# OpenNLPLab/ACR_WSSS

Measured on AMD Instinct MI355X. Metric: img/s ACR-ViT-hybrid-base 448x448 train step, higher is better.
Workload: dtype f32_split; 1 GPU; BASELINE configs[1]: ViT-hybrid-base (DPT) 448x448, batch 16 per GPU, ACR train step (2 views, fwd+bwd+SGD); global_batch=16, classes=20, alpha=125, parallelism=dp1

## Files before the change

acr_wsss_amd/csrc/gemm_f32.hip:

```cpp
#include <math.h>

#include <mutex>
#include <type_traits>
#include <unordered_map>

#include "acr_common.h"

typedef __bf16 bf16_t;

#define F_BM 128
#define F_BN 128
#define F_BK 32
#define F_PKC 36
#define F_PKS 128
#define F_STAGE (F_BM * F_PKC)

struct GemmF32Args {
    const float* a; int64_t lda;
    const float* b; int64_t ldb;
    const float* bias;
    const float* aux; int64_t ldaux;
    float* c; int64_t ldc;
    float* c2;
    float* cs;
    int M, N, K;
    int tiles_m, tiles_n, nsplit, kps;
    int tile0, tiles_launch;
    int nkb_a, nkb_b;
    int img_nkb;
    const int* ea; const int* eb;
    int64_t a_zs, b_zs, c_zs, aux_zs;
    int k_zs, ksplit;
};

#define F_BAND 8
__device__ __forceinline__ void tile_coords(int tt, int tiles_m, int tiles_n, int& tm, int& tn) {
    const int per_band = F_BAND * tiles_n;
    const int band = tt / per_band, in_band = tt - band * per_band;
    const int first = band * F_BAND;
    const int rows = min(tiles_m - first, F_BAND);
    tn = in_band / rows;
    tm = first + (in_band - tn * rows);
}

template <bool KC>
__device__ __forceinline__ void load_chunk(f32x4 (&r)[4], const float* __restrict__ p, int64_t ld, int i0, int dim, int k0,
                                           int kend, int tid) {
#pragma unroll
    for (int ps = 0; ps < 4; ++ps) {
        const int f = tid + 256 * ps;
        if (KC) {
            const int i = min(i0 + (f >> 3), dim - 1), k = min(k0 + 4 * (f & 7), kend - 4);
            r[ps] = *reinterpret_cast<const f32x4*>(p + (int64_t)i * ld + k);
        } else {
            const int k = min(k0 + (f >> 5), kend - 1), i = min(i0 + 4 * (f & 31), dim - 4);
            r[ps] = *reinterpret_cast<const f32x4*>(p + (int64_t)k * ld + i);
        }
    }
}

template <bool KC>
__device__ __forceinline__ void store_chunk(float* __restrict__ s, f32x4 (&r)[4], int k0, int kend, int tid) {
    const f32x4 z = {0.f, 0.f, 0.f, 0.f};
#pragma unroll
    for (int ps = 0; ps < 4; ++ps) {
        const int f = tid + 256 * ps;
        if (KC) {
            if (k0 + 4 * (f & 7) >= kend) r[ps] = z;
            *reinterpret_cast<f32x4*>(s + (f >> 3) * F_PKC + 4 * (f & 7)) = r[ps];
        } else {
            if (k0 + (f >> 5) >= kend) r[ps] = z;
            *reinterpret_cast<f32x4*>(s + (f >> 5) * F_PKS + 4 * (f & 31)) = r[ps];
        }
    }
}

template <bool KC>
__device__ __forceinline__ f32x4 read_frag(const float* __restrict__ s, int base, int q, int r, int h) {
    if (KC) return *reinterpret_cast<const f32x4*>(s + (base + r) * F_PKC + 8 * q + 4 * h);
    const float* p = s + (8 * q + 4 * h) * F_PKS + base + r;
    f32x4 v = {p[0], p[F_PKS], p[2 * F_PKS], p[3 * F_PKS]};
    return v;
}

template <int ACT, bool EDGE>
__device__ __forceinline__ void epilogue_f32(const GemmF32Args& g, f32x16 (&acc)[2][2], int mb, int nb, int r, int h) {
#pragma unroll
    for (int j = 0; j < 2; ++j) {
        const int col = nb + j * 32 + r;
        const bool cok = !EDGE || col < g.N;
        const float bj = (ACT != 2 && g.bias && cok) ? g.bias[col] : 0.f;
#pragma unroll
        for (int i = 0; i < 2; ++i) {
            float x[16];
            if (ACT == 2 || (ACT == 0 && g.aux)) {
#pragma unroll
                for (int e = 0; e < 16; ++e) {
                    const int row = mb + i * 32 + acr_krow(e, h);
                    x[e] = (!EDGE || (row < g.M && cok)) ? g.aux[(int64_t)row * g.ldaux + col] : 0.f;
                }
            }
#pragma unroll
            for (int e = 0; e < 16; ++e) {
                const int row = mb + i * 32 + acr_krow(e, h);
                if (EDGE && !(row < g.M && cok)) continue;
                float v = acc[i][j][e] + bj;
                float* cp = g.c + (int64_t)row * g.ldc + col;
                if (ACT == 0) {
                    *cp = g.aux ? v + x[e] : v;
                } else if (ACT == 1) {
                    const float er = erff(v * 0.70710678118654752440f);
                    g.c2[(int64_t)row * g.ldc + col] = v * 0.5f * (1.0f + er);
                    *cp = 0.5f * (1.0f + er) + v * (expf(-0.5f * v * v) * 0.39894228040143267794f);
                } else {
                    *cp = v * x[e];
                }
            }
        }
    }
}

template <bool A_KC, bool B_KC, int ACT>
__global__ __launch_bounds__(256, 2) void gemm_f32_kernel(const GemmF32Args g) {
    __shared__ __attribute__((aligned(16))) float smem[4 * F_STAGE];
    const int tid = threadIdx.x, lane = tid & 63, wave = tid >> 6;
    const int r = lane & 31, h = lane >> 5, wm = wave >> 1, wn = wave & 1;
    const int ntile = g.tiles_launch;
    const int t = acr_xcd_remap(blockIdx.x, ntile * g.nsplit);
    const int split = t / ntile, tt = g.tile0 + (t - split * ntile);
    int tm, tn;
    if (ACT == 3) { tm = tt / g.tiles_n; tn = tt - tm * g.tiles_n; }
    else tile_coords(tt, g.tiles_m, g.tiles_n, tm, tn);
    const int m0 = tm * F_BM, n0 = tn * F_BN;
    const int zs = split / g.ksplit;
    const int kbeg = (split - zs * g.ksplit) * g.k_zs, kend = min(g.K, kbeg + g.kps);
    const float* __restrict__ pa = g.a + (int64_t)zs * g.a_zs;
    const float* __restrict__ pb = g.b + (int64_t)zs * g.b_zs;

    f32x16 acc[2][2];
#pragma unroll
    for (int i = 0; i < 2; ++i)
#pragma unroll
        for (int j = 0; j < 2; ++j)
#pragma unroll
            for (int e = 0; e < 16; ++e) acc[i][j][e] = 0.f;

    f32x4 ra0[4], rb0[4], ra1[4], rb1[4];
    float csum[4] = {0.f, 0.f, 0.f, 0.f};
    const bool want_cs = ACT == 3 && !A_KC && g.cs && tn == 0;
    auto add_cs = [&](f32x4 (&x)[4]) {
#pragma unroll
        for (int ps = 0; ps < 4; ++ps)
#pragma unroll
            for (int e = 0; e < 4; ++e) csum[e] += x[ps][e];
    };
    auto compute = [&](int buf) {
        const float* sa = smem + buf * 2 * F_STAGE;
        const float* sb = sa + F_STAGE;
#pragma unroll
        for (int q = 0; q < 4; ++q) {
            f32x4 av[2], bv[2];
#pragma unroll
            for (int i = 0; i < 2; ++i) av[i] = read_frag<A_KC>(sa, wm * 64 + i * 32, q, r, h);
#pragma unroll
            for (int j = 0; j < 2; ++j) bv[j] = read_frag<B_KC>(sb, wn * 64 + j * 32, q, r, h);
#pragma unroll
            for (int s = 0; s < 4; ++s)
#pragma unroll
                for (int i = 0; i < 2; ++i)
#pragma unroll
                    for (int j = 0; j < 2; ++j)
                        acc[i][j] = __builtin_amdgcn_mfma_f32_32x32x2f32(av[i][s], bv[j][s], acc[i][j], 0, 0, 0);
        }
    };
    auto step = [&](f32x4 (&la)[4], f32x4 (&lb)[4], f32x4 (&sa_)[4], f32x4 (&sb_)[4], int k0, int buf) {
        if (k0 + 2 * F_BK < kend) {
            load_chunk<A_KC>(la, pa, g.lda, m0, g.M, k0 + 2 * F_BK, kend, tid);
            load_chunk<B_KC>(lb, pb, g.ldb, n0, g.N, k0 + 2 * F_BK, kend, tid);
        }
        compute(buf);
        if (k0 + F_BK < kend) {
            float* d = smem + (buf ^ 1) * 2 * F_STAGE;
            store_chunk<A_KC>(d, sa_, k0 + F_BK, kend, tid);
            store_chunk<B_KC>(d + F_STAGE, sb_, k0 + F_BK, kend, tid);
            if (want_cs) add_cs(sa_);
        }
        __syncthreads();
    };
    load_chunk<A_KC>(ra0, pa, g.lda, m0, g.M, kbeg, kend, tid);
    load_chunk<B_KC>(rb0, pb, g.ldb, n0, g.N, kbeg, kend, tid);
    if (kbeg + F_BK < kend) {
        load_chunk<A_KC>(ra1, pa, g.lda, m0, g.M, kbeg + F_BK, kend, tid);
        load_chunk<B_KC>(rb1, pb, g.ldb, n0, g.N, kbeg + F_BK, kend, tid);
    }
    store_chunk<A_KC>(smem, ra0, kbeg, kend, tid);
    store_chunk<B_KC>(smem + F_STAGE, rb0, kbeg, kend, tid);
    if (want_cs) add_cs(ra0);
    __syncthreads();
    for (int k0 = kbeg; k0 < kend; k0 += 2 * F_BK) {
        step(ra0, rb0, ra1, rb1, k0, 0);
        if (k0 + F_BK < kend) step(ra1, rb1, ra0, rb0, k0 + F_BK, 1);
    }

    if (ACT == 3) {
        float* slab = g.c + (int64_t)split * g.M * g.ldc;
#pragma unroll
        for (int i = 0; i < 2; ++i)
#pragma unroll
            for (int j = 0; j < 2; ++j) {
                const int col = n0 + wn * 64 + j * 32 + r;
#pragma unroll
                for (int e = 0; e < 16; ++e) {
                    const int row = m0 + wm * 64 + i * 32 + acr_krow(e, h);
                    if (row < g.M && col < g.N) slab[(int64_t)row * g.ldc + col] = acc[i][j][e];
                }
            }
        if (!A_KC && g.cs && tn == 0) {
            float* red = smem;
            *reinterpret_cast<f32x4*>(red + (tid >> 5) * 128 + 4 * (tid & 31)) = *reinterpret_cast<f32x4*>(csum);
            __syncthreads();
            if (tid < 128) {
                float s = 0.f;
#pragma unroll
                for (int kr = 0; kr < 8; ++kr) s += red[kr * 128 + tid];
                if (m0 + tid < g.M) g.cs[(int64_t)split * g.M + m0 + tid] = s;
            }
        }
        return;
    }
    GemmF32Args gz = g;
    gz.c += (int64_t)zs * g.c_zs;
    if (gz.aux) gz.aux += (int64_t)zs * g.aux_zs;
    if (m0 + F_BM <= g.M && n0 + F_BN <= g.N)
        epilogue_f32<ACT, false>(gz, acc, m0 + wm * 64, n0 + wn * 64, r, h);
    else
        epilogue_f32<ACT, true>(gz, acc, m0 + wm * 64, n0 + wn * 64, r, h);
}


#define F_DTILE (F_BM * F_BK)

template <bool KC>
__device__ __forceinline__ void dma_offsets(int (&off)[4], int64_t ld, int i0, int dim, int wave, int lane) {
#pragma unroll
    for (int i = 0; i < 4; ++i) {
        const int piece = wave * 4 + i;
        if (KC) {
            const int row = piece * 8 + (lane >> 3);
            const int lc = (lane & 7) ^ ((row >> 1) & 7);
            off[i] = min(i0 + row, dim - 1) * (int)ld + lc * 4;
        } else {
            const int kr = piece * 2 + (lane >> 5);
            off[i] = kr * (int)ld + min(i0 + 4 * (lane & 31), dim - 4);
        }
    }
}
__device__ __forceinline__ void dma_chunk(float* s, const float* __restrict__ ub, const int (&off)[4], int wave) {
    typedef __attribute__((address_space(3))) void* lds_vp;
    typedef const __attribute__((address_space(1))) void* glb_vp;
#pragma unroll
    for (int i = 0; i < 4; ++i)
        __builtin_amdgcn_global_load_lds((glb_vp)(ub + off[i]), (lds_vp)(s + (wave * 4 + i) * 256), 16, 0, 0);
}

template <bool KC>
__device__ __forceinline__ f32x4 dma_frag(const float* __restrict__ s, int base, int q, int r, int h) {
    if (KC) {
        const int row = base + r;
        return *reinterpret_cast<const f32x4*>(s + row * F_BK + (((2 * q + h) ^ ((row >> 1) & 7)) << 2));
    }
    const float* p = s + (8 * q + 4 * h) * F_BM + base + r;
    f32x4 v = {p[0], p[F_BM], p[2 * F_BM], p[3 * F_BM]};
    return v;
}


template <bool A_KC, int ACT>
__device__ __forceinline__ void gemm_f32_finish(const GemmF32Args& g, f32x16 (&acc)[2][2], float* smem, int split, int tt, int tn, int m0,
                                                int n0, int zs, int wm, int wn, int r, int h, int tid, float csum, bool want_cs) {
    if (ACT == 4) {
        float* slab = g.c + ((int64_t)split * g.tiles_launch + (tt - g.tile0)) * (F_BM * F_BN);
#pragma unroll
        for (int i = 0; i < 2; ++i)
#pragma unroll
            for (int j = 0; j < 2; ++j) {
                const int col = wn * 64 + j * 32 + r;
#pragma unroll
                for (int e = 0; e < 16; ++e) slab[(wm * 64 + i * 32 + acr_krow(e, h)) * F_BN + col] = acc[i][j][e];
            }
        return;
    }
    if (ACT == 3) {
        float* slab = g.c + (int64_t)split * g.M * g.ldc;
#pragma unroll
        for (int i = 0; i < 2; ++i)
#pragma unroll
            for (int j = 0; j < 2; ++j) {
                const int col = n0 + wn * 64 + j * 32 + r;
#pragma unroll
                for (int e = 0; e < 16; ++e) {
                    const int row = m0 + wm * 64 + i * 32 + acr_krow(e, h);
                    if (row < g.M && col < g.N) slab[(int64_t)row * g.ldc + col] = acc[i][j][e];
                }
            }
        if (want_cs) {
            float* red = smem;
            red[tid] = csum;
            __syncthreads();
            if (tid < 128 && m0 + tid < g.M) g.cs[(int64_t)split * g.M + m0 + tid] = red[tid] + red[tid + 128];
        }
        return;
    }
    GemmF32Args gz = g;
    gz.c += (int64_t)zs * g.c_zs;
    if (gz.aux) gz.aux += (int64_t)zs * g.aux_zs;
    if (m0 + F_BM <= g.M && n0 + F_BN <= g.N)
        epilogue_f32<ACT, false>(gz, acc, m0 + wm * 64, n0 + wn * 64, r, h);
    else
        epilogue_f32<ACT, true>(gz, acc, m0 + wm * 64, n0 + wn * 64, r, h);
}

template <bool A_KC, bool B_KC, int ACT>
__global__ __launch_bounds__(256, 2) void gemm_f32_dma_kernel(const GemmF32Args g) {
    __shared__ __attribute__((aligned(1024))) float smem[4 * F_DTILE];
    const int tid = threadIdx.x, lane = tid & 63;
    const int wave = __builtin_amdgcn_readfirstlane(tid >> 6);
    const int r = lane & 31, h = lane >> 5, wm = wave >> 1, wn = wave & 1;
    const int ntile = g.tiles_launch;
    const int t = acr_xcd_remap(blockIdx.x, ntile * g.nsplit);
    const int split = t / ntile, tt = g.tile0 + (t - split * ntile);
    int tm, tn;
    if (ACT == 3) { tm = tt / g.tiles_n; tn = tt - tm * g.tiles_n; }
    else tile_coords(tt, g.tiles_m, g.tiles_n, tm, tn);
    const int m0 = tm * F_BM, n0 = tn * F_BN;
    const int zs = split / g.ksplit;
    const int kbeg = (split - zs * g.ksplit) * g.k_zs, kend = min(g.K, kbeg + g.kps);
    const float* __restrict__ pa = g.a + (int64_t)zs * g.a_zs;
    const float* __restrict__ pb = g.b + (int64_t)zs * g.b_zs;
    f32x16 acc[2][2];
#pragma unroll
    for (int i = 0; i < 2; ++i)
#pragma unroll
        for (int j = 0; j < 2; ++j)
#pragma unroll
            for (int e = 0; e < 16; ++e) acc[i][j][e] = 0.f;
    float csum = 0.f;
    const bool want_cs = ACT == 3 && !A_KC && g.cs && tn == 0;

    int offa[4], offb[4];
    dma_offsets<A_KC>(offa, g.lda, m0, g.M, wave, lane);
    dma_offsets<B_KC>(offb, g.ldb, n0, g.N, wave, lane);
    const int64_t ka = A_KC ? 1 : g.lda, kb = B_KC ? 1 : g.ldb;
    dma_chunk(smem, pa + kbeg * ka, offa, wave);
    dma_chunk(smem + F_DTILE, pb + kbeg * kb, offb, wave);
    acr_dma_barrier();
    int cur = 0;
    for (int k0 = kbeg; k0 < kend; k0 += F_BK, cur ^= 1) {
        if (k0 + F_BK < kend) {
            float* d = smem + (cur ^ 1) * 2 * F_DTILE;
            dma_chunk(d, pa + (k0 + F_BK) * ka, offa, wave);
            dma_chunk(d + F_DTILE, pb + (k0 + F_BK) * kb, offb, wave);
        }
// ... 517 lines not shown
    for (int i = 0; i < 2 * NP; ++i) {
        const int q = (wave & 1) * 2 * NP + i, pl = q >> 2, fs = min(f0 + 2 * (q & 3) + (lane >> 5), nkb - 1);
        offd[i] = (fs * NP + pl) * P_TILE_B + (lane & 31) * 16;
    }
    f32x16 acc[2][2];
#pragma unroll
    for (int i = 0; i < 2; ++i)
#pragma unroll
        for (int j = 0; j < 2; ++j)
#pragma unroll
            for (int e = 0; e < 16; ++e) acc[i][j][e] = 0.f;
    const int nst = (kend - kbeg) / P_BK;
    char* sm = reinterpret_cast<char*>(smem);
    auto dma1 = [&](int st, int slot, int i) {
        const int tk = kbeg + st * P_BK;
        const char* src = pw + ((int64_t)(tk >> 7) * nkb) * (NP * P_TILE_B) + (tk & 127) * 32;
        const int q = (wave & 1) * 2 * NP + i;
        __builtin_amdgcn_global_load_lds((glb_vp)(src + offd[i]), (lds_vp)(sm + slot * STAGE_B + (wave >> 1) * (NP * P_TILE_B) + (q >> 2) * P_TILE_B + (q & 3) * 1024),
                                         16, 0, 0);
    };
    const uint32_t lbase = (uint32_t)(uintptr_t)(const __attribute__((address_space(3))) char*)sm;
    const int i16 = lane & 15, g1 = (lane >> 4) & 1, qq = i16 >> 2, pp = i16 & 3;
    const uint32_t tlo = (4 * h + qq) * 32 + ((pp >> 1) << 4) + 8 * (pp & 1), thi = (8 + 4 * h + qq) * 32 + (((pp >> 1) ^ 1) << 4) + 8 * (pp & 1);
    const uint32_t fa_lo = lbase + (wm * 4 + g1) * 512 + tlo, fa_hi = lbase + (wm * 4 + g1) * 512 + thi;
    const uint32_t fb_lo = lbase + NP * P_TILE_B + (wn * 4 + g1) * 512 + tlo, fb_hi = lbase + NP * P_TILE_B + (wn * 4 + g1) * 512 + thi;
#pragma unroll
    for (int i = 0; i < 2 * NP; ++i) dma1(0, 0, i);
#pragma unroll
    for (int i = 0; i < 2 * NP; ++i) dma1(min(1, nst - 1), 1, i);
    bf16x4 al[2][2][NP], ah[2][2][NP], bl[2][2][NP], bh[2][2][NP];
    auto step = [&](int st, int slot, auto set_tag, auto first_tag) {
        constexpr int SET = decltype(set_tag)::value;
        constexpr bool FIRST = decltype(first_tag)::value;
        if constexpr (NP == 3) asm volatile("s_waitcnt vmcnt(6)" ::: "memory");
        else asm volatile("s_waitcnt vmcnt(4)" ::: "memory");
        acr_barrier_nofence();
        const int rslot = slot == 0 ? 2 : slot - 1;
        const int rst = min(st + 2, nst - 1);
        const uint32_t so = slot * STAGE_B;
        const uint32_t a_lo = fa_lo + so, a_hi = fa_hi + so, b_lo = fb_lo + so, b_hi = fb_hi + so;
#define PT_GROUP(K12)                                                                                                                   \
        if constexpr ((K12) < NG) {                                                                                                     \
            if constexpr (!FIRST) pt_mfmas<FMT, (K12) * NM / NG, ((K12) + 1) * NM / NG>(acc, al[SET ^ 1], ah[SET ^ 1], bl[SET ^ 1], bh[SET ^ 1]); \
            if constexpr ((K12) < 2 * NP) PL_RDTR(al[SET][(K12) / NP][(K12) % NP], ah[SET][(K12) / NP][(K12) % NP], a_lo, a_hi, ((K12) % NP) * P_TILE_B + ((K12) / NP) * 1024); \
            else PL_RDTR(bl[SET][((K12) - 2 * NP) / NP][(K12) % NP], bh[SET][((K12) - 2 * NP) / NP][(K12) % NP], b_lo, b_hi, ((K12) % NP) * P_TILE_B + (((K12) - 2 * NP) / NP) * 1024); \
            if ((K12) & 1) dma1(rst, rslot, (K12) >> 1);                                                                                \
            __builtin_amdgcn_sched_barrier(0);                                                                                          \
        }
        PT_GROUP(0) PT_GROUP(1) PT_GROUP(2) PT_GROUP(3) PT_GROUP(4) PT_GROUP(5)
        PT_GROUP(6) PT_GROUP(7) PT_GROUP(8) PT_GROUP(9) PT_GROUP(10) PT_GROUP(11)
#undef PT_GROUP
        if constexpr (NP == 3)
            asm volatile("s_waitcnt lgkmcnt(0)"
                         : "+v"(al[SET][0][0]), "+v"(al[SET][0][1]), "+v"(al[SET][0][2]), "+v"(al[SET][1][0]), "+v"(al[SET][1][1]), "+v"(al[SET][1][2]),
                           "+v"(ah[SET][0][0]), "+v"(ah[SET][0][1]), "+v"(ah[SET][0][2]), "+v"(ah[SET][1][0]), "+v"(ah[SET][1][1]), "+v"(ah[SET][1][2]),
                           "+v"(bl[SET][0][0]), "+v"(bl[SET][0][1]), "+v"(bl[SET][0][2]), "+v"(bl[SET][1][0]), "+v"(bl[SET][1][1]), "+v"(bl[SET][1][2]),
                           "+v"(bh[SET][0][0]), "+v"(bh[SET][0][1]), "+v"(bh[SET][0][2]), "+v"(bh[SET][1][0]), "+v"(bh[SET][1][1]), "+v"(bh[SET][1][2]));
        else
            asm volatile("s_waitcnt lgkmcnt(0)"
                         : "+v"(al[SET][0][0]), "+v"(al[SET][0][1]), "+v"(al[SET][1][0]), "+v"(al[SET][1][1]),
                           "+v"(ah[SET][0][0]), "+v"(ah[SET][0][1]), "+v"(ah[SET][1][0]), "+v"(ah[SET][1][1]),
                           "+v"(bl[SET][0][0]), "+v"(bl[SET][0][1]), "+v"(bl[SET][1][0]), "+v"(bl[SET][1][1]),
                           "+v"(bh[SET][0][0]), "+v"(bh[SET][0][1]), "+v"(bh[SET][1][0]), "+v"(bh[SET][1][1]));
    };
    step(0, 0, std::integral_constant<int, 0>{}, std::true_type{});
    int slot = 1;
    for (int st = 1; st < nst; st += 2) {
        step(st, slot, std::integral_constant<int, 1>{}, std::false_type{});
        slot = slot == 2 ? 0 : slot + 1;
        if (st + 1 < nst) {
            step(st + 1, slot, std::integral_constant<int, 0>{}, std::false_type{});
            slot = slot == 2 ? 0 : slot + 1;
        }
    }
    if (nst & 1) pt_mfmas<FMT, 0, NM>(acc, al[0], ah[0], bl[0], bh[0]);
    else pt_mfmas<FMT, 0, NM>(acc, al[1], ah[1], bl[1], bh[1]);
    asm volatile("s_waitcnt vmcnt(0)" ::: "memory");
    __syncthreads();
    if constexpr (FMT == 1) h2_unscale(g, acc, m0 + wm * 64, n0 + wn * 64, r, h);
    gemm_f32_finish<true, 3>(g, acc, smem, split, tt, tn, m0, n0, 0, wm, wn, r, h, tid, 0.f, false);
}

#define W_STAGE_B (3 * P_TILE_B + S_TILE * 4)
template <int ACT>
__global__ __launch_bounds__(256, 2) void gemm_f32_wimg_kernel(const GemmF32Args g) {
    __shared__ __attribute__((aligned(1024))) float smem[P_SLOTS * W_STAGE_B / 4];
    typedef __attribute__((address_space(3))) void* lds_vp;
    typedef const __attribute__((address_space(1))) void* glb_vp;
    const int tid = threadIdx.x, lane = tid & 63;
    const int wave = __builtin_amdgcn_readfirstlane(tid >> 6);
    const int r = lane & 31, h = lane >> 5, wm = wave >> 1, wn = wave & 1;
    const int ntile = g.tiles_launch;
    const int t0 = acr_xcd_remap(blockIdx.x, ntile * g.nsplit);
    const int split = t0 / ntile, tt = g.tile0 + (t0 - split * ntile);
    int tm, tn;
    if (ACT == 3) { tm = tt / g.tiles_n; tn = tt - tm * g.tiles_n; }
    else tile_coords(tt, g.tiles_m, g.tiles_n, tm, tn);
    const int m0 = tm * F_BM, n0 = tn * F_BN;
    const int zs = split / g.ksplit;
    const int kbeg = (split - zs * g.ksplit) * g.k_zs, kend = min(g.K, kbeg + g.kps);
    const int nkb = (g.K + P_BK - 1) / P_BK;
    const char* __restrict__ pa = reinterpret_cast<const char*>(g.a) + ((int64_t)tm * nkb + kbeg / P_BK) * (3 * P_TILE_B) + wave * 3072 + lane * 16;
    const float* __restrict__ pb = g.b + (int64_t)zs * g.b_zs + (int64_t)kbeg * g.ldb;
    int offb[2];
#pragma unroll
    for (int i = 0; i < 2; ++i) offb[i] = ((wave * 2 + i) * 2 + (lane >> 5)) * (int)g.ldb + min(n0 + 4 * (lane & 31), g.N - 4);
    f32x16 acc[2][2];
#pragma unroll
    for (int i = 0; i < 2; ++i)
#pragma unroll
        for (int j = 0; j < 2; ++j)
#pragma unroll
            for (int e = 0; e < 16; ++e) acc[i][j][e] = 0.f;
    const int nst = (kend - kbeg) / P_BK;
    char* sm = reinterpret_cast<char*>(smem);
    auto dma1 = [&](int st, int slot, int i) {
        if (i < 3)
            __builtin_amdgcn_global_load_lds((glb_vp)(pa + (int64_t)st * (3 * P_TILE_B) + i * 1024), (lds_vp)(sm + slot * W_STAGE_B + (wave * 3 + i) * 1024), 16, 0, 0);
        else
            __builtin_amdgcn_global_load_lds((glb_vp)(pb + (int64_t)st * P_BK * g.ldb + offb[i - 3]),
                                             (lds_vp)(sm + slot * W_STAGE_B + 3 * P_TILE_B + (wave * 2 + i - 3) * 1024), 16, 0, 0);
    };
    const uint32_t lbase = (uint32_t)(uintptr_t)(const __attribute__((address_space(3))) char*)sm;
    const uint32_t fa = lbase + (wm * 64 + r) * 32 + (h ^ ((r >> 3) & 1)) * 16;
    const uint32_t fb = lbase + 3 * P_TILE_B + ((8 * h) * F_BN + wn * 64 + r) * 4;
#pragma unroll
    for (int i = 0; i < 5; ++i) dma1(0, 0, i);
#pragma unroll
    for (int i = 0; i < 5; ++i) dma1(min(1, nst - 1), 1, i);
    bf16x8 ap[2][2][3], bp[2][2][3];
    float rb[2][8];
#define WI_MFMA6(SET, I, J)                                                                                                  \
    acc[I][J] = __builtin_amdgcn_mfma_f32_32x32x16_bf16(ap[SET][I][0], bp[SET][J][2], acc[I][J], 0, 0, 0);                   \
    acc[I][J] = __builtin_amdgcn_mfma_f32_32x32x16_bf16(ap[SET][I][2], bp[SET][J][0], acc[I][J], 0, 0, 0);                   \
    acc[I][J] = __builtin_amdgcn_mfma_f32_32x32x16_bf16(ap[SET][I][1], bp[SET][J][1], acc[I][J], 0, 0, 0);                   \
    acc[I][J] = __builtin_amdgcn_mfma_f32_32x32x16_bf16(ap[SET][I][0], bp[SET][J][1], acc[I][J], 0, 0, 0);                   \
    acc[I][J] = __builtin_amdgcn_mfma_f32_32x32x16_bf16(ap[SET][I][1], bp[SET][J][0], acc[I][J], 0, 0, 0);                   \
    acc[I][J] = __builtin_amdgcn_mfma_f32_32x32x16_bf16(ap[SET][I][0], bp[SET][J][0], acc[I][J], 0, 0, 0);
#define WI_RD32(dst, addr, OFF) asm volatile("ds_read_b32 %0, %1 offset:%2" : "=&v"(dst) : "v"(addr), "i"(OFF))
    auto step = [&](int st, int slot, auto set_tag, auto first_tag) {
        constexpr int SET = decltype(set_tag)::value;
        constexpr bool FIRST = decltype(first_tag)::value;
        asm volatile("s_waitcnt vmcnt(5)" ::: "memory");
        acr_barrier_nofence();
        const int rslot = slot == 0 ? 2 : slot - 1;
        const int rst = min(st + 2, nst - 1);
#pragma unroll
        for (int i = 0; i < 5; ++i) dma1(rst, rslot, i);
        const uint32_t fas = fa + slot * W_STAGE_B, fbs = fb + slot * W_STAGE_B;
#pragma unroll
        for (int j = 0; j < 2; ++j) {
            WI_RD32(rb[j][0], fbs, 0 * F_BN * 4 + j * 128); WI_RD32(rb[j][1], fbs, 1 * F_BN * 4 + j * 128); WI_RD32(rb[j][2], fbs, 2 * F_BN * 4 + j * 128);
            WI_RD32(rb[j][3], fbs, 3 * F_BN * 4 + j * 128); WI_RD32(rb[j][4], fbs, 4 * F_BN * 4 + j * 128); WI_RD32(rb[j][5], fbs, 5 * F_BN * 4 + j * 128);
            WI_RD32(rb[j][6], fbs, 6 * F_BN * 4 + j * 128); WI_RD32(rb[j][7], fbs, 7 * F_BN * 4 + j * 128);
        }
#pragma unroll
        for (int i = 0; i < 2; ++i) {
            PL_RD(ap[SET][i][0], fas, 0 * P_TILE_B + i * 1024); PL_RD(ap[SET][i][1], fas, 1 * P_TILE_B + i * 1024); PL_RD(ap[SET][i][2], fas, 2 * P_TILE_B + i * 1024);
        }
        asm volatile("s_waitcnt lgkmcnt(6)" : "+v"(rb[0][0]), "+v"(rb[0][1]), "+v"(rb[0][2]), "+v"(rb[0][3]), "+v"(rb[0][4]), "+v"(rb[0][5]), "+v"(rb[0][6]),
                     "+v"(rb[0][7]), "+v"(rb[1][0]), "+v"(rb[1][1]), "+v"(rb[1][2]), "+v"(rb[1][3]), "+v"(rb[1][4]), "+v"(rb[1][5]), "+v"(rb[1][6]), "+v"(rb[1][7]));
        __builtin_amdgcn_sched_barrier(0);
#pragma unroll
        for (int j = 0; j < 2; ++j) {
            const f32x4 lo = {rb[j][0], rb[j][1], rb[j][2], rb[j][3]}, hi = {rb[j][4], rb[j][5], rb[j][6], rb[j][7]};
            split3_bf16(lo, hi, bp[SET][j][0], bp[SET][j][1], bp[SET][j][2]);
        }
        if (!FIRST) {
            WI_MFMA6(SET ^ 1, 0, 0) WI_MFMA6(SET ^ 1, 0, 1) WI_MFMA6(SET ^ 1, 1, 0) WI_MFMA6(SET ^ 1, 1, 1)
#pragma unroll
            for (int it = 0; it < 24; ++it) {
                __builtin_amdgcn_sched_group_barrier(0x008, 1, 0);
                __builtin_amdgcn_sched_group_barrier(0x002, 4, 0);
            }
        }
        __builtin_amdgcn_sched_barrier(0);
        asm volatile("s_waitcnt lgkmcnt(0)" : "+v"(ap[SET][0][0]), "+v"(ap[SET][0][1]), "+v"(ap[SET][0][2]), "+v"(ap[SET][1][0]), "+v"(ap[SET][1][1]), "+v"(ap[SET][1][2]));
    };
    step(0, 0, std::integral_constant<int, 0>{}, std::true_type{});
    int slot = 1;
    for (int st = 1; st < nst; st += 2) {
        step(st, slot, std::integral_constant<int, 1>{}, std::false_type{});
        slot = slot == 2 ? 0 : slot + 1;
        if (st + 1 < nst) {
            step(st + 1, slot, std::integral_constant<int, 0>{}, std::false_type{});
            slot = slot == 2 ? 0 : slot + 1;
        }
    }
    if (nst & 1) { WI_MFMA6(0, 0, 0) WI_MFMA6(0, 0, 1) WI_MFMA6(0, 1, 0) WI_MFMA6(0, 1, 1) }
    else { WI_MFMA6(1, 0, 0) WI_MFMA6(1, 0, 1) WI_MFMA6(1, 1, 0) WI_MFMA6(1, 1, 1) }
#undef WI_MFMA6
    asm volatile("s_waitcnt vmcnt(0)" ::: "memory");
    __syncthreads();
    gemm_f32_finish<true, ACT>(g, acc, smem, split, tt, tn, m0, n0, zs, wm, wn, r, h, tid, 0.f, false);
}

#define W64_BN 256
#define W64_A_B (3 * 2048)
#define W64_STAGE_B (W64_A_B + P_BK * W64_BN * 4)
template <int ACT>
__global__ __launch_bounds__(256, 2) void gemm_f32_wimg64_kernel(const GemmF32Args g) {
    __shared__ __attribute__((aligned(1024))) char sm[P_SLOTS * W64_STAGE_B];
    typedef __attribute__((address_space(3))) void* lds_vp;
    typedef const __attribute__((address_space(1))) void* glb_vp;
    const int tid = threadIdx.x, lane = tid & 63;
    const int wave = __builtin_amdgcn_readfirstlane(tid >> 6);
    const int r = lane & 31, h = lane >> 5, wn = wave;
    const int ntile = g.tiles_n;
    const int t0 = acr_xcd_remap(blockIdx.x, ntile * g.nsplit);
    const int split = t0 / ntile, tn = t0 - split * ntile;
    const int n0 = tn * W64_BN;
    const int zs = split / g.ksplit;
    const int kbeg = (split - zs * g.ksplit) * g.k_zs, kend = min(g.K, kbeg + g.kps);
    const int qa = wave < 3 ? 2 * wave : 4;
    const char* __restrict__ pa = reinterpret_cast<const char*>(g.a) + (int64_t)(kbeg / P_BK) * (3 * P_TILE_B) + lane * 16;
    const float* __restrict__ pb = g.b + (int64_t)zs * g.b_zs + (int64_t)kbeg * g.ldb + min(n0 + 4 * lane, g.N - 4);
    f32x16 acc[2][2];
#pragma unroll
    for (int i = 0; i < 2; ++i)
#pragma unroll
        for (int j = 0; j < 2; ++j)
#pragma unroll
            for (int e = 0; e < 16; ++e) acc[i][j][e] = 0.f;
    const int nst = (kend - kbeg) / P_BK;
    auto issue = [&](int st, int slot) {
        char* d = sm + slot * W64_STAGE_B;
#pragma unroll
        for (int i = 0; i < 2; ++i) {
            const int q = qa + i;
            __builtin_amdgcn_global_load_lds((glb_vp)(pa + (int64_t)st * (3 * P_TILE_B) + (q >> 1) * P_TILE_B + (q & 1) * 1024), (lds_vp)(d + q * 1024), 16, 0, 0);
        }
#pragma unroll
        for (int i = 0; i < 4; ++i)
            __builtin_amdgcn_global_load_lds((glb_vp)(pb + (int64_t)(st * P_BK + 4 * wave + i) * g.ldb), (lds_vp)(d + W64_A_B + (4 * wave + i) * 1024), 16, 0, 0);
    };
    const uint32_t lbase = (uint32_t)(uintptr_t)(const __attribute__((address_space(3))) char*)sm;
    const uint32_t fa = lbase + r * 32 + (h ^ ((r >> 3) & 1)) * 16;
    const uint32_t fb = lbase + W64_A_B + ((8 * h) * W64_BN + wn * 64 + r) * 4;
    issue(0, 0);
    issue(min(1, nst - 1), 1);
    bf16x8 ap[2][2][3], bp[2][2][3];
    float rb[2][8];
#define W64_MFMA6(SET, I, J)                                                                                                 \
    acc[I][J] = __builtin_amdgcn_mfma_f32_32x32x16_bf16(ap[SET][I][0], bp[SET][J][2], acc[I][J], 0, 0, 0);                   \
    acc[I][J] = __builtin_amdgcn_mfma_f32_32x32x16_bf16(ap[SET][I][2], bp[SET][J][0], acc[I][J], 0, 0, 0);                   \
    acc[I][J] = __builtin_amdgcn_mfma_f32_32x32x16_bf16(ap[SET][I][1], bp[SET][J][1], acc[I][J], 0, 0, 0);                   \
    acc[I][J] = __builtin_amdgcn_mfma_f32_32x32x16_bf16(ap[SET][I][0], bp[SET][J][1], acc[I][J], 0, 0, 0);                   \
    acc[I][J] = __builtin_amdgcn_mfma_f32_32x32x16_bf16(ap[SET][I][1], bp[SET][J][0], acc[I][J], 0, 0, 0);                   \
    acc[I][J] = __builtin_amdgcn_mfma_f32_32x32x16_bf16(ap[SET][I][0], bp[SET][J][0], acc[I][J], 0, 0, 0);
#define W64_RD32(dst, addr, OFF) asm volatile("ds_read_b32 %0, %1 offset:%2" : "=&v"(dst) : "v"(addr), "i"(OFF))
    auto step = [&](int st, int slot, auto set_tag, auto first_tag) {
        constexpr int SET = decltype(set_tag)::value;
        constexpr bool FIRST = decltype(first_tag)::value;
        asm volatile("s_waitcnt vmcnt(6)" ::: "memory");
        acr_barrier_nofence();
        const int rslot = slot == 0 ? 2 : slot - 1;
        issue(min(st + 2, nst - 1), rslot);
        const uint32_t fas = fa + slot * W64_STAGE_B, fbs = fb + slot * W64_STAGE_B;
#pragma unroll
        for (int j = 0; j < 2; ++j) {
            W64_RD32(rb[j][0], fbs, 0 * W64_BN * 4 + j * 128); W64_RD32(rb[j][1], fbs, 1 * W64_BN * 4 + j * 128);
            W64_RD32(rb[j][2], fbs, 2 * W64_BN * 4 + j * 128); W64_RD32(rb[j][3], fbs, 3 * W64_BN * 4 + j * 128);
            W64_RD32(rb[j][4], fbs, 4 * W64_BN * 4 + j * 128); W64_RD32(rb[j][5], fbs, 5 * W64_BN * 4 + j * 128);
            W64_RD32(rb[j][6], fbs, 6 * W64_BN * 4 + j * 128); W64_RD32(rb[j][7], fbs, 7 * W64_BN * 4 + j * 128);
        }
#pragma unroll
        for (int i = 0; i < 2; ++i) {
            PL_RD(ap[SET][i][0], fas, 0 * 2048 + i * 1024); PL_RD(ap[SET][i][1], fas, 1 * 2048 + i * 1024); PL_RD(ap[SET][i][2], fas, 2 * 2048 + i * 1024);
        }
        asm volatile("s_waitcnt lgkmcnt(6)" : "+v"(rb[0][0]), "+v"(rb[0][1]), "+v"(rb[0][2]), "+v"(rb[0][3]), "+v"(rb[0][4]), "+v"(rb[0][5]), "+v"(rb[0][6]),
                     "+v"(rb[0][7]), "+v"(rb[1][0]), "+v"(rb[1][1]), "+v"(rb[1][2]), "+v"(rb[1][3]), "+v"(rb[1][4]), "+v"(rb[1][5]), "+v"(rb[1][6]), "+v"(rb[1][7]));
        __builtin_amdgcn_sched_barrier(0);
#pragma unroll
        for (int j = 0; j < 2; ++j) {
            const f32x4 lo = {rb[j][0], rb[j][1], rb[j][2], rb[j][3]}, hi = {rb[j][4], rb[j][5], rb[j][6], rb[j][7]};
            split3_bf16(lo, hi, bp[SET][j][0], bp[SET][j][1], bp[SET][j][2]);
        }
// ... 783 lines not shown
            hipLaunchKernelGGL((gemm_f32_split_kernel<false, false, 3>), dim3((unsigned)(g.tiles_m * g.tiles_n * p.nsplit)), dim3(256), 0, st, g);
        else if ((K % F_BK) == 0 && off32_ok(M, N, K, lda, ldb, mode))
            hipLaunchKernelGGL((gemm_f32_dma_kernel<false, false, 3>), dim3((unsigned)(g.tiles_m * g.tiles_n * p.nsplit)), dim3(256), 0, st, g);
        else
            hipLaunchKernelGGL((gemm_f32_kernel<false, false, 3>), dim3((unsigned)(g.tiles_m * g.tiles_n * p.nsplit)), dim3(256), 0, st, g);
        const int64_t n4 = (int64_t)M * N / 4;
        hipLaunchKernelGGL(gemm_f32_reduce_kernel, dim3((unsigned)((n4 + 255) / 256)), dim3(256), 0, st, (const float*)ws, p.nsplit, n4, c);
        if (colsum)
            hipLaunchKernelGGL(gemm_f32_reduce1_kernel, dim3((M + 255) / 256), dim3(256), 0, st, (const float*)g.cs, p.nsplit, M, colsum);
        return acr_check_launch("acr_gemm_f32(TN)");
    }
    ACR_CHECK_ARG((K % 4) == 0 && K >= 4, "acr_gemm_f32: NT / NN need K %% 4 == 0 (K=%d)", K);
    if (mode == ACR_GEMM_NN) ACR_CHECK_ARG((N % 4) == 0 && N >= 4, "acr_gemm_f32: NN needs N %% 4 == 0 (N=%d)", N);
    ACR_CHECK_ARG(act != 1 || c2, "acr_gemm_f32: act 1 (GELU) needs c2");
    ACR_CHECK_ARG(act != 2 || aux, "acr_gemm_f32: act 2 (GELU') needs the saved pre-activation in aux");
#define ACR_F32_LAUNCH(AK, BK_, ACTV)                                                                              \
    do {                                                                                                            \
        if (dma && split) hipLaunchKernelGGL((gemm_f32_split_kernel<AK, BK_, ACTV>), grid, dim3(256), 0, st, g);   \
        else if (dma) hipLaunchKernelGGL((gemm_f32_dma_kernel<AK, BK_, ACTV>), grid, dim3(256), 0, st, g);          \
        else hipLaunchKernelGGL((gemm_f32_kernel<AK, BK_, ACTV>), grid, dim3(256), 0, st, g);                      \
    } while (0)
    const bool split = math == ACR_MATH_BF16X3;
    const bool dma = (K % F_BK) == 0 && off32_ok(M, N, K, lda, ldb, mode);
    TailPlan tp = gemm_tail_plan(M, N, K);
    const bool vec_ok = al16(c) && (ldc % 4) == 0 && (!bias || al16(bias)) && (!aux || (al16(aux) && (ldaux % 4) == 0)) &&
                        (!c2 || al16(c2));
    if (!dma || !ws || !al16(ws) || !vec_ok) tp.ntail = 0;
    if (tp.ntail) {
        g.tiles_launch -= tp.ntail;
        grid = dim3((unsigned)g.tiles_launch);
    }
    const PlanesPlan pl = planes_plan(mode, math, M, N, K);
    if (math == ACR_MATH_FP16X2) {
        ACR_CHECK_ARG(ws && al16(ws) && vec_ok, "acr_gemm_f32: fp16x2 needs the acr_gemm_f32_ws_floats workspace (16-byte aligned) and 16-byte aligned c / bias / aux / c2");
        float* pa = ws + (gemm_ws_base_floats(mode, M, N, K, true) + 3) / 4 * 4;
        float* pb = pa + pl.a_fl;
        h2_image_rows(a, lda, M, K, pa, nullptr, nullptr, st);
        if (mode == ACR_GEMM_NT) h2_image_rows(b, ldb, N, K, pb, nullptr, nullptr, st);
        else h2_image_t(b, ldb, K, N, pb, pb + pl.b_fl, st);
        return gemm_planes<1>(ACR_GEMM_NT, act, pa, pb, bias, aux, ldaux, c, ldc, c2, nullptr, M, N, K, ws, h2_exps(pa, M, K), h2_exps(pb, N, K), st);
    }
    if (pl.on && ws && al16(ws) && vec_ok) {
        float* wp = ws + (gemm_ws_base_floats(mode, M, N, K, true) + 3) / 4 * 4;
        float* pa = wp;
        float* pb = wp + pl.a_fl;
        int rc = acr_x3_image(a, lda, M, K, pa, nullptr, nullptr, stream);
        if (rc == ACR_OK) rc = mode == ACR_GEMM_NT ? acr_x3_image(b, ldb, N, K, pb, nullptr, nullptr, stream) : acr_x3_image_t(b, ldb, K, N, pb, stream);
        if (rc == ACR_OK) rc = acr_gemm_x3(ACR_GEMM_NT, act, pa, pb, bias, aux, ldaux, c, ldc, c2, nullptr, M, N, K, ws, stream);
        return rc;
    }
    if (g.tiles_launch == 0) {
    } else if (mode == ACR_GEMM_NT) {
        if (act == 0) ACR_F32_LAUNCH(true, true, 0);
        else if (act == 1) ACR_F32_LAUNCH(true, true, 1);
        else ACR_F32_LAUNCH(true, true, 2);
    } else {
        if (act == 0) ACR_F32_LAUNCH(true, false, 0);
        else if (act == 1) ACR_F32_LAUNCH(true, false, 1);
        else ACR_F32_LAUNCH(true, false, 2);
    }
#undef ACR_F32_LAUNCH
    if (tp.ntail) {
        GemmF32Args gt = g;
        gt.tile0 = g.tiles_launch; gt.tiles_launch = tp.ntail; gt.nsplit = tp.nsplit; gt.kps = tp.kps; gt.k_zs = tp.kps;
        gt.c = ws;
        const dim3 tgrid((unsigned)(tp.ntail * tp.nsplit));
        if (mode == ACR_GEMM_NT && split) hipLaunchKernelGGL((gemm_f32_split_kernel<true, true, 4>), tgrid, dim3(256), 0, st, gt);
        else if (mode == ACR_GEMM_NT) hipLaunchKernelGGL((gemm_f32_dma_kernel<true, true, 4>), tgrid, dim3(256), 0, st, gt);
        else if (split) hipLaunchKernelGGL((gemm_f32_split_kernel<true, false, 4>), tgrid, dim3(256), 0, st, gt);
        else hipLaunchKernelGGL((gemm_f32_dma_kernel<true, false, 4>), tgrid, dim3(256), 0, st, gt);
        GemmF32Args ge = g;
        ge.tile0 = gt.tile0;
        const dim3 egrid((unsigned)(tp.ntail * 16));
        if (act == 0) hipLaunchKernelGGL((gemm_f32_tail_epilogue_kernel<0>), egrid, dim3(256), 0, st, ge, (const float*)ws, tp.ntail, tp.nsplit);
        else if (act == 1) hipLaunchKernelGGL((gemm_f32_tail_epilogue_kernel<1>), egrid, dim3(256), 0, st, ge, (const float*)ws, tp.ntail, tp.nsplit);
        else hipLaunchKernelGGL((gemm_f32_tail_epilogue_kernel<2>), egrid, dim3(256), 0, st, ge, (const float*)ws, tp.ntail, tp.nsplit);
    }
    return acr_check_launch("acr_gemm_f32");
}

static void conv_args(GemmF32Args& g, int M, int N, int K) {
    g.bias = nullptr; g.aux = nullptr; g.ldaux = 0; g.c2 = nullptr; g.cs = nullptr; g.M = M; g.N = N; g.K = K;
    g.tiles_m = (M + F_BM - 1) / F_BM; g.tiles_n = (N + F_BN - 1) / F_BN; g.kps = (K + F_BK - 1) / F_BK * F_BK; g.k_zs = 0;
    g.a_zs = g.b_zs = g.c_zs = g.aux_zs = 0; g.ksplit = 1;
    g.tile0 = 0; g.tiles_launch = g.tiles_m * g.tiles_n;
}

static int conv1x1_ksplit(int nsamp, int cout, int cin, int hw, int* kps_out, bool wide64 = false) {
    const int tiles = wide64 ? ((hw + 255) / 256) * nsamp : ((cout + F_BM - 1) / F_BM) * ((hw + F_BN - 1) / F_BN) * nsamp;
    *kps_out = (cin + S_BK - 1) / S_BK * S_BK;
    if (tiles >= 192 || (cin % F_BK) != 0) return 1;
    int ks = 512 / tiles;
    if (ks > cin / 64) ks = cin / 64;
    if (ks < 2) return 1;
    const int kps = ((cin + ks - 1) / ks + S_BK - 1) / S_BK * S_BK;
    *kps_out = kps;
    return (cin + kps - 1) / kps;
}
extern "C" size_t acr_conv1x1_ws_floats(int32_t math, int32_t nsamp, int32_t cout, int32_t cin, int32_t hw) {
    int kps;
    if (math != ACR_MATH_BF16X3) return 0;
    int ks = conv1x1_ksplit(nsamp, cout, cin, hw, &kps);
    if (cout <= 64) ks = max(ks, conv1x1_ksplit(nsamp, cout, cin, hw, &kps, true));
    return ks > 1 ? (size_t)ks * nsamp * cout * hw : 0;
}
__global__ __launch_bounds__(256) void conv1x1_ksum_kernel(const float* __restrict__ ws, int ks, int64_t per4, const float* __restrict__ addend,
                                                           float* __restrict__ y, int64_t n4) {
    const int64_t i = (int64_t)blockIdx.x * 256 + threadIdx.x;
    if (i >= n4) return;
    const int64_t n = i / per4, e = i - n * per4;
    const f32x4* p = reinterpret_cast<const f32x4*>(ws) + n * ks * per4 + e;
    f32x4 s = p[0];
    for (int k = 1; k < ks; ++k) {
        const f32x4 v = p[(int64_t)k * per4];
        s[0] += v[0]; s[1] += v[1]; s[2] += v[2]; s[3] += v[3];
    }
    if (addend) {
        const f32x4 v = reinterpret_cast<const f32x4*>(addend)[i];
        s[0] += v[0]; s[1] += v[1]; s[2] += v[2]; s[3] += v[3];
    }
    reinterpret_cast<f32x4*>(y)[i] = s;
}

extern "C" int acr_conv1x1_f32(int32_t math, const float* w, int32_t w_transposed, const float* x, const float* addend, float* y, int32_t nsamp,
                               int32_t cout, int32_t cin, int32_t hw, float* ws, void* stream) {
    ACR_CHECK_ARG(w && x && y, "acr_conv1x1_f32: null pointer");
    ACR_CHECK_ARG(nsamp > 0 && cout > 0 && cin > 0 && hw > 0 && (hw % 4) == 0 && (cin % 4) == 0 && (cout % 4) == 0,
                  "acr_conv1x1_f32: need hw, cin, cout %% 4 == 0 (n=%d co=%d ci=%d hw=%d)", nsamp, cout, cin, hw);
    ACR_CHECK_ARG(al16(w) && al16(x) && al16(y) && al16(addend), "acr_conv1x1_f32: 16-byte alignment");
    hipStream_t st = (hipStream_t)stream;
    GemmF32Args g;
    conv_args(g, cout, hw, cin);
    g.a = w; g.b = x; g.ldb = hw; g.b_zs = (int64_t)cin * hw;
    g.c = y; g.ldc = hw; g.c_zs = (int64_t)cout * hw;
    g.aux = addend; g.ldaux = hw; g.aux_zs = (int64_t)cout * hw;
    g.nsplit = nsamp;
    const dim3 grid((unsigned)(g.tiles_m * g.tiles_n * nsamp));
    const bool dma = (cin % F_BK) == 0;
    if (math == ACR_MATH_FP16X2) {
        acr_set_error("acr_conv1x1_f32: ACR_MATH_FP16X2 is built for the block Linears only (acr_gemm_f32)");
        return ACR_ERR_UNSUPPORTED;
    }
    ACR_CHECK_ARG(math == ACR_MATH_F32 || math == ACR_MATH_BF16X3, "acr_conv1x1_f32: bad math %d", math);
    const bool split = dma && math == ACR_MATH_BF16X3;
    int kps = 0;
    const int ks = (split && ws && al16(ws)) ? conv1x1_ksplit(nsamp, cout, cin, hw, &kps) : 1;
    if (ks > 1) {
        g.lda = w_transposed ? cout : cin;
        g.nsplit = nsamp * ks; g.ksplit = ks; g.kps = kps; g.k_zs = kps;
        g.c = ws; g.ldc = hw; g.aux = nullptr;
        const dim3 kgrid((unsigned)(g.tiles_m * g.tiles_n * nsamp * ks));
        if (!w_transposed) hipLaunchKernelGGL((gemm_f32_split_kernel<true, false, 3>), kgrid, dim3(256), 0, st, g);
        else hipLaunchKernelGGL((gemm_f32_split_kernel<false, false, 3>), kgrid, dim3(256), 0, st, g);
        const int64_t per4 = (int64_t)cout * hw / 4, n4 = per4 * nsamp;
        hipLaunchKernelGGL(conv1x1_ksum_kernel, dim3((unsigned)((n4 + 255) / 256)), dim3(256), 0, st, (const float*)ws, ks, per4, addend, y, n4);
        return acr_check_launch("acr_conv1x1_f32(K-split)");
    }
    if (!w_transposed) {
        g.lda = cin;
        if (split) hipLaunchKernelGGL((gemm_f32_split_kernel<true, false, 0>), grid, dim3(256), 0, st, g);
        else if (dma) hipLaunchKernelGGL((gemm_f32_dma_kernel<true, false, 0>), grid, dim3(256), 0, st, g);
        else hipLaunchKernelGGL((gemm_f32_kernel<true, false, 0>), grid, dim3(256), 0, st, g);
    } else {
        g.lda = cout;
        if (split) hipLaunchKernelGGL((gemm_f32_split_kernel<false, false, 0>), grid, dim3(256), 0, st, g);
        else if (dma) hipLaunchKernelGGL((gemm_f32_dma_kernel<false, false, 0>), grid, dim3(256), 0, st, g);
        else hipLaunchKernelGGL((gemm_f32_kernel<false, false, 0>), grid, dim3(256), 0, st, g);
    }
    return acr_check_launch("acr_conv1x1_f32");
}

extern "C" int acr_conv1x1_x3(const float* w_img, const float* x, const float* addend, float* y, int32_t nsamp, int32_t cout, int32_t cin,
                              int32_t hw, float* ws, void* stream) {
    ACR_CHECK_ARG(w_img && x && y, "acr_conv1x1_x3: null pointer");
    ACR_CHECK_ARG(nsamp > 0 && cout > 0 && cin > 0 && hw >= 4 && (hw % 4) == 0 && (cin % P_BK) == 0 && (cout % 4) == 0,
                  "acr_conv1x1_x3: need hw, cout %% 4 == 0, cin %% 16 == 0 (n=%d co=%d ci=%d hw=%d)", nsamp, cout, cin, hw);
    ACR_CHECK_ARG(al16(w_img) && al16(x) && al16(y) && al16(addend), "acr_conv1x1_x3: 16-byte alignment");
    ACR_CHECK_ARG((int64_t)cin * hw < (1ll << 30), "acr_conv1x1_x3: sample too large for 32-bit offsets");
    hipStream_t st = (hipStream_t)stream;
    GemmF32Args g;
    conv_args(g, cout, hw, cin);
    g.a = w_img; g.lda = 0; g.b = x; g.ldb = hw; g.b_zs = (int64_t)cin * hw;
    g.c = y; g.ldc = hw; g.c_zs = (int64_t)cout * hw;
    g.aux = addend; g.ldaux = hw; g.aux_zs = (int64_t)cout * hw;
    g.nsplit = nsamp; g.kps = cin; g.k_zs = 0;
    const bool wide64 = cout <= 64 && hw >= 4;
    if (wide64) { g.tiles_m = 1; g.tiles_n = (hw + W64_BN - 1) / W64_BN; g.tiles_launch = g.tiles_n; }
    int kps = 0;
    const int ks = (ws && al16(ws)) ? conv1x1_ksplit(nsamp, cout, cin, hw, &kps, wide64) : 1;
    if (ks > 1) {
        g.nsplit = nsamp * ks; g.ksplit = ks; g.kps = kps; g.k_zs = kps;
        g.c = ws; g.aux = nullptr;
        if (wide64) hipLaunchKernelGGL((gemm_f32_wimg64_kernel<3>), dim3((unsigned)(g.tiles_n * nsamp * ks)), dim3(256), 0, st, g);
        else
        hipLaunchKernelGGL((gemm_f32_wimg_kernel<3>), dim3((unsigned)(g.tiles_m * g.tiles_n * nsamp * ks)), dim3(256), 0, st, g);
        const int64_t per4 = (int64_t)cout * hw / 4, n4 = per4 * nsamp;
        hipLaunchKernelGGL(conv1x1_ksum_kernel, dim3((unsigned)((n4 + 255) / 256)), dim3(256), 0, st, (const float*)ws, ks, per4, addend, y, n4);
        return acr_check_launch("acr_conv1x1_x3(K-split)");
    }
    if (wide64) hipLaunchKernelGGL((gemm_f32_wimg64_kernel<0>), dim3((unsigned)(g.tiles_n * nsamp)), dim3(256), 0, st, g);
    else hipLaunchKernelGGL((gemm_f32_wimg_kernel<0>), dim3((unsigned)(g.tiles_m * g.tiles_n * nsamp)), dim3(256), 0, st, g);
    return acr_check_launch("acr_conv1x1_x3");
}

static int conv_wgrad_ksplit(int nsamp, int cout, int cin, int hw) {
    const int tiles = ((cout + F_BM - 1) / F_BM) * ((cin + F_BN - 1) / F_BN) * nsamp;
    int ks = 512 / tiles;
    const int maxs = hw / 512;
    if (ks > maxs) ks = maxs;
    if (ks < 1) ks = 1;
    const int kps = ((hw + ks - 1) / ks + F_BK - 1) / F_BK * F_BK;
    return (hw + kps - 1) / kps;
}
extern "C" size_t acr_conv1x1_wgrad_f32_ws_floats(int32_t nsamp, int32_t cout, int32_t cin, int32_t hw) {
    return (size_t)nsamp * conv_wgrad_ksplit(nsamp, cout, cin, hw) * cout * cin;
}

extern "C" int acr_conv1x1_wgrad_f32(int32_t math, const float* dy, const float* x, int32_t nsamp, int32_t cout, int32_t cin, int32_t hw, float* ws,
                                     float* dw, void* stream) {
    ACR_CHECK_ARG(dy && x && ws && dw, "acr_conv1x1_wgrad_f32: null pointer");
    ACR_CHECK_ARG(nsamp > 0 && cout > 0 && cin > 0 && hw > 0 && (hw % 4) == 0 && (cin % 4) == 0 && (cout % 4) == 0,
                  "acr_conv1x1_wgrad_f32: need hw, cin, cout %% 4 == 0");
    ACR_CHECK_ARG(al16(dy) && al16(x) && al16(dw) && al16(ws), "acr_conv1x1_wgrad_f32: 16-byte alignment");
    hipStream_t st = (hipStream_t)stream;
    GemmF32Args g;
    conv_args(g, cout, cin, hw);
    g.a = dy; g.lda = hw; g.a_zs = (int64_t)cout * hw;
    g.b = x; g.ldb = hw; g.b_zs = (int64_t)cin * hw;
    g.c = ws; g.ldc = cin;
    const int ks = conv_wgrad_ksplit(nsamp, cout, cin, hw);
    g.ksplit = ks;
    g.kps = ((hw + ks - 1) / ks + F_BK - 1) / F_BK * F_BK;
    ACR_CHECK_ARG((int64_t)(ks - 1) * g.kps < hw, "acr_conv1x1_wgrad_f32: internal split plan");
    g.k_zs = g.kps;
    g.nsplit = nsamp * ks;
    const dim3 grid((unsigned)(g.tiles_m * g.tiles_n * g.nsplit));
    if (math == ACR_MATH_FP16X2) {
        acr_set_error("acr_conv1x1_wgrad_f32: ACR_MATH_FP16X2 is built for the block Linears only (acr_gemm_f32)");
        return ACR_ERR_UNSUPPORTED;
    }
    ACR_CHECK_ARG(math == ACR_MATH_F32 || math == ACR_MATH_BF16X3, "acr_conv1x1_wgrad_f32: bad math %d", math);
    if ((hw % S_BK) == 0 && math == ACR_MATH_BF16X3)
        hipLaunchKernelGGL((gemm_f32_split_kernel<true, true, 3>), grid, dim3(256), 0, st, g);
    else if ((hw % F_BK) == 0)
        hipLaunchKernelGGL((gemm_f32_dma_kernel<true, true, 3>), grid, dim3(256), 0, st, g);
    else
        hipLaunchKernelGGL((gemm_f32_kernel<true, true, 3>), grid, dim3(256), 0, st, g);
    const int64_t n4 = (int64_t)cout * cin / 4;
    if (!acr_slab_sum_wide(ws, g.nsplit, n4, dw, st))
        hipLaunchKernelGGL(gemm_f32_reduce_kernel, dim3((unsigned)((n4 + 255) / 256)), dim3(256), 0, st, (const float*)ws, g.nsplit, n4, dw);
    return acr_check_launch("acr_conv1x1_wgrad_f32");
}
```

Baseline: 129.6 img/s.

## Flatten batch and pixel dims into GEMM columns for 1x1 conv forward

For the non-split 1x1 conv path, the per-sample grid is replaced by one GEMM whose N dimension spans all samples' pixels. B-operand column offsets and a new NCHW epilogue map each flattened column back to its sample and pixel. This removes partial edge tiles per sample when hw is not a multiple of the tile width, and gives a single larger launch. The cost is a per-column divide, and loads of four consecutive columns that cross a sample boundary may be read incorrectly unless hw is a multiple of 4.

```diff
diff --git a/acr_wsss_amd/csrc/gemm_f32.hip b/acr_wsss_amd/csrc/gemm_f32.hip
--- a/acr_wsss_amd/csrc/gemm_f32.hip
+++ b/acr_wsss_amd/csrc/gemm_f32.hip
@@ -31,6 +31,7 @@
     const int* ea; const int* eb;
     int64_t a_zs, b_zs, c_zs, aux_zs;
     int k_zs, ksplit;
+    int hw;
 };
 
 #define F_BAND 8
@@ -115,6 +116,37 @@
                 } else {
                     *cp = v * x[e];
                 }
+            }
+        }
+    }
+}
+
+template <bool EDGE>
+__device__ __forceinline__ void epilogue_nchw(const GemmF32Args& g, f32x16 (&acc)[2][2], int mb, int nb, int r, int h) {
+#pragma unroll
+    for (int j = 0; j < 2; ++j) {
+        const int col = nb + j * 32 + r;
+        const bool cok = !EDGE || col < g.N;
+        const int cc = cok ? col : 0, n = cc / g.hw, p = cc - n * g.hw;
+        float* __restrict__ cb = g.c + (int64_t)n * g.c_zs + p;
+        const float* __restrict__ ab = g.aux ? g.aux + (int64_t)n * g.aux_zs + p : nullptr;
+        const float bj = 0.f;
+#pragma unroll
+        for (int i = 0; i < 2; ++i) {
+            float x[16];
+            if (ab) {
+#pragma unroll
+                for (int e = 0; e < 16; ++e) {
+                    const int row = mb + i * 32 + acr_krow(e, h);
+                    x[e] = (!EDGE || (row < g.M && cok)) ? ab[(int64_t)row * g.ldaux] : 0.f;
+                }
+            }
+#pragma unroll
+            for (int e = 0; e < 16; ++e) {
+                const int row = mb + i * 32 + acr_krow(e, h);
+                if (EDGE && !(row < g.M && cok)) continue;
+                const float v = acc[i][j][e] + bj;
+                cb[(int64_t)row * g.ldc] = ab ? v + x[e] : v;
             }
         }
     }
@@ -275,9 +307,17 @@
 }
 
 
-template <bool A_KC, int ACT>
+template <bool A_KC, int ACT, bool FLAT = false>
 __device__ __forceinline__ void gemm_f32_finish(const GemmF32Args& g, f32x16 (&acc)[2][2], float* smem, int split, int tt, int tn, int m0,
                                                 int n0, int zs, int wm, int wn, int r, int h, int tid, float csum, bool want_cs) {
+    static_assert(!FLAT || ACT == 0, "flattened pixel columns: plain epilogue only");
+    if constexpr (FLAT) {
+        if (m0 + F_BM <= g.M && n0 + F_BN <= g.N)
+            epilogue_nchw<false>(g, acc, m0 + wm * 64, n0 + wn * 64, r, h);
+        else
+            epilogue_nchw<true>(g, acc, m0 + wm * 64, n0 + wn * 64, r, h);
+        return;
+    }
     if (ACT == 4) {
         float* slab = g.c + ((int64_t)split * g.tiles_launch + (tt - g.tile0)) * (F_BM * F_BN);
 #pragma unroll
@@ -961,8 +1001,9 @@
 }
 
 #define W_STAGE_B (3 * P_TILE_B + S_TILE * 4)
-template <int ACT>
+template <int ACT, bool FLAT = false>
 __global__ __launch_bounds__(256, 2) void gemm_f32_wimg_kernel(const GemmF32Args g) {
+    static_assert(!FLAT || ACT == 0, "flattened pixel columns: plain epilogue only");
     __shared__ __attribute__((aligned(1024))) float smem[P_SLOTS * W_STAGE_B / 4];
     typedef __attribute__((address_space(3))) void* lds_vp;
     typedef const __attribute__((address_space(1))) void* glb_vp;
@@ -982,8 +1023,13 @@
     const char* __restrict__ pa = reinterpret_cast<const char*>(g.a) + ((int64_t)tm * nkb + kbeg / P_BK) * (3 * P_TILE_B) + wave * 3072 + lane * 16;
     const float* __restrict__ pb = g.b + (int64_t)zs * g.b_zs + (int64_t)kbeg * g.ldb;
     int offb[2];
-#pragma unroll
-    for (int i = 0; i < 2; ++i) offb[i] = ((wave * 2 + i) * 2 + (lane >> 5)) * (int)g.ldb + min(n0 + 4 * (lane & 31), g.N - 4);
+    int pcol = min(n0 + 4 * (lane & 31), g.N - 4);
+    if (FLAT) {
+        const int n = pcol / g.hw;
+        pcol = n * (int)g.b_zs + (pcol - n * g.hw);
+    }
+#pragma unroll
+    for (int i = 0; i < 2; ++i) offb[i] = ((wave * 2 + i) * 2 + (lane >> 5)) * (int)g.ldb + pcol;
     f32x16 acc[2][2];
 #pragma unroll
     for (int i = 0; i < 2; ++i)
@@ -1071,7 +1117,7 @@
 #undef WI_MFMA6
     asm volatile("s_waitcnt vmcnt(0)" ::: "memory");
     __syncthreads();
-    gemm_f32_finish<true, ACT>(g, acc, smem, split, tt, tn, m0, n0, zs, wm, wn, r, h, tid, 0.f, false);
+    gemm_f32_finish<true, ACT, FLAT>(g, acc, smem, split, tt, tn, m0, n0, zs, wm, wn, r, h, tid, 0.f, false);
 }
 
 #define W64_BN 256
@@ -2021,7 +2067,7 @@
 static void conv_args(GemmF32Args& g, int M, int N, int K) {
     g.bias = nullptr; g.aux = nullptr; g.ldaux = 0; g.c2 = nullptr; g.cs = nullptr; g.M = M; g.N = N; g.K = K;
     g.tiles_m = (M + F_BM - 1) / F_BM; g.tiles_n = (N + F_BN - 1) / F_BN; g.kps = (K + F_BK - 1) / F_BK * F_BK; g.k_zs = 0;
-    g.a_zs = g.b_zs = g.c_zs = g.aux_zs = 0; g.ksplit = 1;
+    g.a_zs = g.b_zs = g.c_zs = g.aux_zs = 0; g.ksplit = 1; g.hw = 0;
     g.tile0 = 0; g.tiles_launch = g.tiles_m * g.tiles_n;
 }
 
@@ -2138,7 +2184,11 @@
         return acr_check_launch("acr_conv1x1_x3(K-split)");
     }
     if (wide64) hipLaunchKernelGGL((gemm_f32_wimg64_kernel<0>), dim3((unsigned)(g.tiles_n * nsamp)), dim3(256), 0, st, g);
-    else hipLaunchKernelGGL((gemm_f32_wimg_kernel<0>), dim3((unsigned)(g.tiles_m * g.tiles_n * nsamp)), dim3(256), 0, st, g);
+    else if ((int64_t)nsamp * cin * hw < (1ll << 31)) {
+        g.hw = hw; g.N = nsamp * hw; g.nsplit = 1;
+        g.tiles_n = (g.N + F_BN - 1) / F_BN; g.tiles_launch = g.tiles_m * g.tiles_n;
+        hipLaunchKernelGGL((gemm_f32_wimg_kernel<0, true>), dim3((unsigned)g.tiles_launch), dim3(256), 0, st, g);
+    } else hipLaunchKernelGGL((gemm_f32_wimg_kernel<0>), dim3((unsigned)(g.tiles_m * g.tiles_n * nsamp)), dim3(256), 0, st, g);
     return acr_check_launch("acr_conv1x1_x3");
 }
 
```

New measurement: 129.8 img/s, median of 6. About the same (+0.2%).
